# leavesnight/VIEO_SLAM

Measured on AMD Instinct MI355X. Metric: frontend+localBA frames/sec on EuRoC MH05 stereo-VIO; ATE vs ref, higher is better.
Workload: dtype u8 (extract/match) + f64 (pose optimisation)

## Files before the change

vieo_slam_amd/csrc/orb_extractor.hip:

```cpp
#include <algorithm>
#include <cmath>
#include <type_traits>
#include <vector>

#include "../../include/vieo_orb_pattern_31.h"
#include "common.h"
#include "sincosf_exact.h"
#include "wave_ops.h"

#define QT_DEVICE
#include "quadtree.inl"

#include "orb_internal.h"

namespace vieo {

#ifndef VIEO_RESIZE_ROWS
#define VIEO_RESIZE_ROWS 32
#endif
static const int kResizeRows = VIEO_RESIZE_ROWS;
#ifndef VIEO_QT_GROUPS
#define VIEO_QT_GROUPS {1, 64}
#endif

// ... 599 lines not shown
  int pitch;
  const uint8_t* src = plane_ptr(P, I, b, t.level, &pitch);
  const int ox = t.tx * kBlurTW, oy = t.ty * kBlurTH;
  const bool interior = ox >= 4 && ox + 68 <= D.w && oy >= 3 && oy + kBlurTH + 3 <= D.h &&
                        ((pitch & 3) == 0) && ((((uintptr_t)src) & 3) == 0);
  if (interior) {
    constexpr int NIT = (SH * (SP / 4) + 255) / 256;
    unsigned v[NIT];
#pragma unroll
    for (int k = 0; k < NIT; k++) {
      const int idx = tid + 256 * k, r = idx / (SP / 4), c4 = idx - r * (SP / 4);
      if (idx < SH * (SP / 4)) v[k] = *(const unsigned*)(src + (size_t)(oy + r - 3) * pitch + ox - 4 + 4 * c4);
    }
#pragma unroll
    for (int k = 0; k < NIT; k++)
      if (tid + 256 * k < SH * (SP / 4)) ((unsigned*)s_src)[tid + 256 * k] = v[k];
  } else {
    const bool aligned = ((pitch & 3) == 0) && ((((uintptr_t)src) & 3) == 0);
    constexpr int NIT = (SH * (SP / 4) + 255) / 256;
    unsigned v[NIT];
#pragma unroll
    for (int k = 0; k < NIT; k++) {
      const int idx = tid + 256 * k, r = idx / (SP / 4), c4 = idx - r * (SP / 4);
      v[k] = 0;
      if (idx < SH * (SP / 4)) {
        const int gy = reflect101(min(oy + r - 3, D.h + 2), D.h);
        const int gx0 = ox - 4 + 4 * c4;
        const uint8_t* row = src + (size_t)gy * pitch;
        if (aligned && gx0 >= 0 && gx0 + 4 <= D.w)
          v[k] = *(const unsigned*)(row + gx0);
        else {
#pragma unroll
          for (int j = 0; j < 4; j++) v[k] |= (unsigned)row[reflect101(min(gx0 + j, D.w + 2), D.w)] << (8 * j);
        }
      }
    }
#pragma unroll
    for (int k = 0; k < NIT; k++)
      if (tid + 256 * k < SH * (SP / 4)) ((unsigned*)s_src)[tid + 256 * k] = v[k];
  }
  __syncthreads();
  const unsigned K0123 = 18u | (34u << 8) | (48u << 16) | (56u << 24);
  const unsigned K456 = 48u | (34u << 8) | (18u << 16);
#ifndef VIEO_BLUR_AB
#define VIEO_BLUR_AB 0
#endif
  for (int idx = tid; idx < ((VIEO_BLUR_AB & 1) ? 0 : (SH / 2) * (kBlurTW / 4)); idx += 256) {
    const int pr = idx / (kBlurTW / 4), g = idx - pr * (kBlurTW / 4);
    unsigned h[2][4];
#pragma unroll
    for (int q = 0; q < 2; q++) {
      const unsigned* w = (const unsigned*)(s_src + (2 * pr + q) * SP) + g;
      const unsigned w0 = w[0], w1 = w[1], w2 = w[2];
      const unsigned a0 = __builtin_amdgcn_alignbyte(w1, w0, 1), b0 = __builtin_amdgcn_alignbyte(w2, w1, 1);
      const unsigned a1 = __builtin_amdgcn_alignbyte(w1, w0, 2), b1 = __builtin_amdgcn_alignbyte(w2, w1, 2);
      const unsigned a2 = __builtin_amdgcn_alignbyte(w1, w0, 3), b2 = __builtin_amdgcn_alignbyte(w2, w1, 3);
      h[q][0] = __builtin_amdgcn_udot4(b0, K456, __builtin_amdgcn_udot4(a0, K0123, 0u, false), false);
      h[q][1] = __builtin_amdgcn_udot4(b1, K456, __builtin_amdgcn_udot4(a1, K0123, 0u, false), false);
      h[q][2] = __builtin_amdgcn_udot4(b2, K456, __builtin_amdgcn_udot4(a2, K0123, 0u, false), false);
      h[q][3] = __builtin_amdgcn_udot4(w2, K456, __builtin_amdgcn_udot4(w1, K0123, 0u, false), false);
    }
    uint4 o;
    o.x = h[0][0] | (h[1][0] << 16), o.y = h[0][1] | (h[1][1] << 16);
    o.z = h[0][2] | (h[1][2] << 16), o.w = h[0][3] | (h[1][3] << 16);
    *(uint4*)(s_h + pr * kBlurTW + 4 * g) = o;
  }
  __syncthreads();
  typedef unsigned short us2 __attribute__((ext_vector_type(2)));
  uint8_t* dst = I.blur + (size_t)b * I.blur_img + D.boff;
  for (int idx = tid; idx < (kBlurTH / 2) * (kBlurTW / 4); idx += 256) {
    const int q = idx / (kBlurTW / 4), c4 = (idx - q * (kBlurTW / 4)) * 4;
    const int gy = oy + 2 * q, gx = ox + c4;
    if (gy >= D.h || gx >= D.w) continue;
#if VIEO_BLUR_AB & 1
    *(unsigned*)(dst + (size_t)gy * D.pitch + gx) = *(const unsigned*)(s_src + (2 * q + 3) * SP + c4 + 4);
    if (gy + 1 < D.h) *(unsigned*)(dst + (size_t)(gy + 1) * D.pitch + gx) = *(const unsigned*)(s_src + (2 * q + 4) * SP + c4 + 4);
    continue;
#endif
    const unsigned We[4] = {18u | (34u << 16), 48u | (56u << 16), 48u | (34u << 16), 18u};
    const unsigned Wo[4] = {18u << 16, 34u | (48u << 16), 56u | (48u << 16), 34u | (18u << 16)};
    unsigned e[4] = {1u << 15, 1u << 15, 1u << 15, 1u << 15}, o[4] = {1u << 15, 1u << 15, 1u << 15, 1u << 15};
#pragma unroll
    for (int k = 0; k < 4; k++) {
      const uint4 v = *(const uint4*)(s_h + (q + k) * kBlurTW + c4);
      const unsigned vv[4] = {v.x, v.y, v.z, v.w};
#pragma unroll
      for (int j = 0; j < 4; j++) {
        e[j] = __builtin_amdgcn_udot2(__builtin_bit_cast(us2, vv[j]), __builtin_bit_cast(us2, We[k]), e[j], false);
        o[j] = __builtin_amdgcn_udot2(__builtin_bit_cast(us2, vv[j]), __builtin_bit_cast(us2, Wo[k]), o[j], false);
      }
    }
    const unsigned oe = ((e[0] >> 16) & 0xFFu) | (((e[1] >> 16) & 0xFFu) << 8) | (((e[2] >> 16) & 0xFFu) << 16) |
                        (((e[3] >> 16) & 0xFFu) << 24);
    const unsigned oo = ((o[0] >> 16) & 0xFFu) | (((o[1] >> 16) & 0xFFu) << 8) | (((o[2] >> 16) & 0xFFu) << 16) |
                        (((o[3] >> 16) & 0xFFu) << 24);
    *(unsigned*)(dst + (size_t)gy * D.pitch + gx) = oe;
    if (gy + 1 < D.h) *(unsigned*)(dst + (size_t)(gy + 1) * D.pitch + gx) = oo;
  }
}

__device__ __forceinline__ int wave_sum(int v) { return wave_sum_i32(v); }

__device__ __forceinline__ float fast_atan2_deg(float y, float x) {
  const float p1 = 0.9997878412794807f * (float)(180 / 3.1415926535897932384626433832795);
  const float p3 = -0.3258083974640975f * (float)(180 / 3.1415926535897932384626433832795);
  const float p5 = 0.1555786518463281f * (float)(180 / 3.1415926535897932384626433832795);
  const float p7 = -0.04432655554792128f * (float)(180 / 3.1415926535897932384626433832795);
  const float eps = (float)2.2204460492503131e-16;
  const float ax = fabsf(x), ay = fabsf(y);
  float a, c, c2;
  if (ax >= ay) {
    c = ay / (ax + eps);
    c2 = c * c;
    a = (((p7 * c2 + p5) * c2 + p3) * c2 + p1) * c;
  } else {
    c = ax / (ay + eps);
    c2 = c * c;
    a = 90.f - (((p7 * c2 + p5) * c2 + p3) * c2 + p1) * c;
  }
  if (x < 0) a = 180.f - a;
  if (y < 0) a = 360.f - a;
  return a;
}

__global__ void __launch_bounds__(256)
k_desc_index(OrbParams P, const unsigned* __restrict__ sel, const int* __restrict__ sel_count,
             uint2* __restrict__ krec, int out_cap, int* __restrict__ counts) {
  const int b = blockIdx.y, g = blockIdx.x * 256 + threadIdx.x;
  int level = -1, idx = 0, total = 0;
  for (int l = 0; l < P.nlevels; l++) {
    const int n = max(sel_count[b * kMaxLevels + l], 0);
    if (level < 0 && g < total + n) {
      level = l;
      idx = g - total;
    }
    total += n;
  }
  if (g == 0) {
    counts[2 * b] = min(total, out_cap);
    counts[2 * b + 1] = 0;
  }
  if (g >= P.kp_cap) return;
  unsigned key = 0;
  if (level >= 0) key = sel[(size_t)b * P.sel_per_image + P.lv[level].sel_off + idx];
  krec[(size_t)b * P.kp_cap + g] = make_uint2(key, (unsigned)level);
}

#ifndef VIEO_DESC_KPW
#define VIEO_DESC_KPW 1
#endif
__global__ void __launch_bounds__(256)
k_describe(OrbParams P, ImgSet I, const uint2* __restrict__ krec, const int* __restrict__ pattern,
           vieo_keypoint* __restrict__ kp_out, uint8_t* __restrict__ desc_out, int out_cap,
           int groups_per_image, int n_images) {
  constexpr int KPW = VIEO_DESC_KPW;
  const int item = xcd_grouped(blockIdx.x, groups_per_image);
  const int b = item / groups_per_image;
  if (b >= n_images) return;
  const int lane = threadIdx.x & 63;
  const int wv = __builtin_amdgcn_readfirstlane((int)(threadIdx.x >> 6));
  const int g0 = ((item - b * groups_per_image) * (blockDim.x >> 6) + wv) * KPW;
  const int gmax = min(P.kp_cap, out_cap);
  if (g0 >= gmax) return;
  uint2 kr[KPW];
#pragma unroll
  for (int u = 0; u < KPW; u++) kr[u] = g0 + u < gmax ? krec[(size_t)b * P.kp_cap + g0 + u] : make_uint2(0, 0xFFFFFFFFu);
  constexpr int AP = 40, BR = 19, BP = 44;
  __shared__ __attribute__((aligned(16))) uint8_t s_patch[4][KPW][31 * AP + (2 * BR + 1) * BP];
  int pt4[4];
#pragma unroll
  for (int gq = 0; gq < 4; gq++) pt4[gq] = pattern[gq * 64 + lane];
  int cxs[KPW], cys[KPW], xas[KPW], xbs[KPW];
  unsigned va[KPW][8], vb[KPW][10];
  const int c = lane & 15, r0 = lane >> 4;
#pragma unroll
  for (int u = 0; u < KPW; u++) {
    const int level = (int)kr[u].y;
    if (level < 0) continue;
    const unsigned key = kr[u].x;
    const LevelDesc& D = P.lv[level];
    const int cx = QT_KEY_X(key) + (kEdge - 3), cy = QT_KEY_Y(key) + (kEdge - 3);
    int pitch;
    const uint8_t* img = plane_ptr(P, I, b, level, &pitch);
    const int xa = (cx - kHalfPatch) & ~3, xb = (cx - BR) & ~3;
    cxs[u] = cx, cys[u] = cy, xas[u] = xa, xbs[u] = xb;
    const uint8_t* bl0 = I.blur + (size_t)b * I.blur_img + D.boff;
    const int bp = D.pitch;
    const uint8_t* ga = img + (size_t)(cy - kHalfPatch + r0) * pitch + xa + 4 * c;
    const uint8_t* gb = bl0 + (size_t)(cy - BR + r0) * bp + xb + 4 * c;
#pragma unroll
    for (int k = 0; k < 8; k++)
      if (c < 9 && r0 + 4 * k < 31) va[u][k] = *(const unsigned*)(ga + (size_t)(4 * k) * pitch);
#pragma unroll
    for (int k = 0; k < 10; k++)
      if (c < 11 && r0 + 4 * k < 2 * BR + 1) vb[u][k] = *(const unsigned*)(gb + (size_t)(4 * k) * bp);
  }
#pragma unroll
  for (int u = 0; u < KPW; u++) {
    if ((int)kr[u].y < 0) continue;
    uint8_t* sa = s_patch[wv][u];
    uint8_t* sb = sa + 31 * AP;
#pragma unroll
    for (int k = 0; k < 8; k++)
      if (c < 9 && r0 + 4 * k < 31) *(unsigned*)(sa + (r0 + 4 * k) * AP + 4 * c) = va[u][k];
#pragma unroll
    for (int k = 0; k < 10; k++)
      if (c < 11 && r0 + 4 * k < 2 * BR + 1) *(unsigned*)(sb + (r0 + 4 * k) * BP + 4 * c) = vb[u][k];
  }
  __builtin_amdgcn_fence(__ATOMIC_ACQ_REL, "workgroup");
  __builtin_amdgcn_wave_barrier();
#pragma unroll
  for (int u = 0; u < KPW; u++) {
    const int level = (int)kr[u].y;
    if (level < 0) continue;
    const int g = g0 + u;
    const unsigned key = kr[u].x;
    const LevelDesc& D = P.lv[level];
    const int cx = cxs[u], cy = cys[u], xa = xas[u], xb = xbs[u];
    const uint8_t* sa = s_patch[wv][u];
    const uint8_t* sb = sa + 31 * AP;
    int m10 = 0, m01 = 0;
    if (lane < 62) {
      const int v = (lane >> 1) - kHalfPatch;
      const int d = P.umax[v < 0 ? -v : v];
      const uint8_t* row = sa + (v + kHalfPatch) * AP + (cx - xa);
      const int u0 = (lane & 1) ? 0 : -d, u1 = (lane & 1) ? d : -1;
      int sI = 0;
#pragma unroll
      for (int t = 0; t < 16; t++) {
        const int uu = u0 + t;
        if (uu <= u1) {
          const int val = row[uu];
          m10 += uu * val;
          sI += val;
        }
      }
      m01 = v * sI;
    }
    m10 = wave_sum(m10);
    m01 = wave_sum(m01);
    const float angle = fast_atan2_deg((float)m01, (float)m10);
    const float factorPI = (float)(3.1415926535897932384626433832795 / 180.f);
    float a, bsin;
    vieo_sincosf_exact(angle * factorPI, &bsin, &a);
    const uint8_t* bl = sb + BR * BP + (cx - xb);
    unsigned long long bits[4];
#pragma unroll
    for (int gq = 0; gq < 4; gq++) {
      const int pt = pt4[gq];
      const float x0 = (float)(signed char)(pt & 0xFF), y0 = (float)(signed char)((pt >> 8) & 0xFF);
      const float x1 = (float)(signed char)((pt >> 16) & 0xFF), y1 = (float)(signed char)((pt >> 24) & 0xFF);
      const int t0 = bl[__float2int_rn(x0 * bsin + y0 * a) * BP + __float2int_rn(x0 * a - y0 * bsin)];
      const int t1 = bl[__float2int_rn(x1 * bsin + y1 * a) * BP + __float2int_rn(x1 * a - y1 * bsin)];
      bits[gq] = __ballot(t0 < t1);
    }
    if (lane < 4) ((unsigned long long*)(desc_out + ((size_t)b * out_cap + g) * 32))[lane] = bits[lane];
    if (lane == 0) {
      vieo_keypoint k;
      const float fx = (float)cx, fy = (float)cy;
      k.x = level ? fx * D.scale : fx;
      k.y = level ? fy * D.scale : fy;
      k.size = (float)D.patch;
      k.angle = angle;
      k.response = (float)QT_KEY_R(key);
      k.octave = level;
      k.class_id = -1;
      kp_out[(size_t)b * out_cap + g] = k;
    }
  }
}

#ifndef VIEO_FUSED_AB
#define VIEO_FUSED_AB 0
#endif
constexpr int kFR = 18, kFRaw = kFR + 3;
constexpr int kFRawRows = 2 * kFRaw + 1, kFRawPitch = 48;
constexpr int kFHPairs = (kFRawRows + 1) / 2, kFHCols = 40;
constexpr int kFBlRows = 2 * kFR + 1, kFBlPitch = 40;
constexpr int kFWaveLds = kFRawRows * kFRawPitch + 16 + kFHPairs * kFHCols * 4;
static_assert(kFBlRows * kFBlPitch <= kFRawRows * kFRawPitch, "the blurred patch fits where the raw one was");

#ifndef VIEO_FUSED_KPW
#define VIEO_FUSED_KPW 4
#endif
static inline int fused_kpw(int n_images) { return n_images >= 32 ? VIEO_FUSED_KPW : 1; }
__global__ void __launch_bounds__(256)
k_describe_fused(OrbParams P, ImgSet I, const uint2* __restrict__ krec, const int* __restrict__ pattern,
                 vieo_keypoint* __restrict__ kp_out, uint8_t* __restrict__ desc_out, int out_cap,
                 int groups_per_image, int n_images, int KPW) {
  const int item = xcd_grouped(blockIdx.x, groups_per_image);
  const int b = item / groups_per_image;
  if (b >= n_images) return;
  const int lane = threadIdx.x & 63;
  const int wv = __builtin_amdgcn_readfirstlane((int)(threadIdx.x >> 6));
  const int g0 = ((item - b * groups_per_image) * (blockDim.x >> 6) + wv) * KPW;
  const int gmax = min(P.kp_cap, out_cap);
  if (g0 >= gmax) return;
  __shared__ __attribute__((aligned(16))) uint8_t s_all[4][kFWaveLds];
  int pt4[4];
#pragma unroll
  for (int gq = 0; gq < 4; gq++) pt4[gq] = pattern[gq * 64 + lane];
  uint8_t* s_raw = s_all[wv];
  unsigned* s_h = (unsigned*)(s_raw + kFRawRows * kFRawPitch + 16);
  constexpr int NLD = (kFRawRows + 3) / 4;
  unsigned v[NLD];
  bool interior = false;
  int sh = 0;
  const int c = lane & 15, r0 = lane >> 4;
  auto rec_of = [&](int u) { return (u < KPW && g0 + u < gmax) ? krec[(size_t)b * P.kp_cap + g0 + u] : make_uint2(0u, 0xFFFFFFFFu); };
  auto fetch = [&](const uint2 kr) {
    const int level = (int)kr.y;
    if (level < 0) return;
    const LevelDesc& D = P.lv[level];
    const int cx = QT_KEY_X(kr.x) + (kEdge - 3), cy = QT_KEY_Y(kr.x) + (kEdge - 3);
    int pitch;
    const uint8_t* img = plane_ptr(P, I, b, level, &pitch);
    const int x_lo = cx - kFRaw, y_lo = cy - kFRaw;
    const int xa = x_lo & ~3;
    sh = x_lo - xa;
    interior = x_lo >= 0 && y_lo >= 0 && cx + kFRaw < D.w && cy + kFRaw < D.h && xa + 52 <= pitch && ((pitch & 3) == 0) &&
               ((((uintptr_t)img) & 3) == 0);
    if (VIEO_FUSED_AB & 2) {
#pragma unroll
      for (int k = 0; k < NLD; k++) v[k] = kr.x + k;
      interior = false;
    } else if (interior) {
      const uint8_t* gp = img + (size_t)(y_lo + r0) * pitch + xa + 4 * c;
#pragma unroll
      for (int k = 0; k < NLD; k++) {
        v[k] = 0;
        if (c < 13 && r0 + 4 * k < kFRawRows) v[k] = *(const unsigned*)(gp + (size_t)(4 * k) * pitch);
      }
    } else {
#pragma unroll
      for (int k = 0; k < NLD; k++) {
        v[k] = 0;
        if (c < 12 && r0 + 4 * k < kFRawRows) {
          const uint8_t* row = img + (size_t)reflect101(min(max(y_lo + r0 + 4 * k, -(D.h - 1)), 2 * D.h - 2), D.h) * pitch;
#pragma unroll
          for (int jj = 0; jj < 4; jj++) {
            const int x = min(max(x_lo + 4 * c + jj, -(D.w - 1)), 2 * D.w - 2);
            v[k] |= (unsigned)row[reflect101(x, D.w)] << (8 * jj);
          }
        }
      }
    }
  };
  uint2 kr = rec_of(0);
  fetch(kr);
#pragma unroll 1
  for (int u = 0; u < KPW; u++) {
    const uint2 cur = kr;
    const int level = (int)cur.y;
    if (level < 0) break;
    const unsigned key = cur.x;
    const int g = g0 + u;
    const LevelDesc& D = P.lv[level];
    const int cx = QT_KEY_X(key) + (kEdge - 3), cy = QT_KEY_Y(key) + (kEdge - 3);
    if (interior) {
#pragma unroll
      for (int k = 0; k < NLD; k++) {
        const unsigned nxt = (unsigned)__builtin_amdgcn_update_dpp(0, (int)v[k], 0x101, 0xF, 0xF, false);
        v[k] = __builtin_amdgcn_alignbyte(nxt, v[k], sh);
      }
    }
#pragma unroll
    for (int k = 0; k < NLD; k++)
      if (c < 12 && r0 + 4 * k < kFRawRows) *(unsigned*)(s_raw + (r0 + 4 * k) * kFRawPitch + 4 * c) = v[k];
    __builtin_amdgcn_fence(__ATOMIC_ACQ_REL, "workgroup");
    __builtin_amdgcn_wave_barrier();
    kr = rec_of(u + 1);
    fetch(kr);
    {
      constexpr unsigned A0 = 18u | (34u << 8) | (48u << 16) | (56u << 24), A1 = 48u | (34u << 8) | (18u << 16);
      constexpr unsigned B0 = (18u << 8) | (34u << 16) | (48u << 24), B1 = 56u | (48u << 8) | (34u << 16) | (18u << 24);
      constexpr unsigned C0 = (18u << 16) | (34u << 24), C1 = 48u | (56u << 8) | (48u << 16) | (34u << 24), C2 = 18u;
      constexpr unsigned E0 = 18u << 24, E1 = 34u | (48u << 8) | (56u << 16) | (48u << 24), E2 = 34u | (18u << 8);
      for (int idx = lane; idx < ((VIEO_FUSED_AB & 1) ? 0 : kFHPairs * (kFHCols / 8)); idx += 64) {
        const int pr = idx / (kFHCols / 8), g8 = idx - pr * (kFHCols / 8);
        unsigned h[2][8];
#pragma unroll
        for (int q = 0; q < 2; q++) {
          const int r = min(2 * pr + q, kFRawRows - 1);
          const uint2* w = (const uint2*)(s_raw + r * kFRawPitch + 8 * g8);
          const uint2 lo = w[0], hi = w[1];
          const unsigned d0 = lo.x, d1 = lo.y, d2 = hi.x, d3 = hi.y;
#define DOT4(x, k, acc) __builtin_amdgcn_udot4(x, k, acc, false)
          h[q][0] = DOT4(d1, A1, DOT4(d0, A0, 0u));
          h[q][1] = DOT4(d1, B1, DOT4(d0, B0, 0u));
          h[q][2] = DOT4(d2, C2, DOT4(d1, C1, DOT4(d0, C0, 0u)));
          h[q][3] = DOT4(d2, E2, DOT4(d1, E1, DOT4(d0, E0, 0u)));
          h[q][4] = DOT4(d2, A1, DOT4(d1, A0, 0u));
          h[q][5] = DOT4(d2, B1, DOT4(d1, B0, 0u));
          h[q][6] = DOT4(d3, C2, DOT4(d2, C1, DOT4(d1, C0, 0u)));
          h[q][7] = DOT4(d3, E2, DOT4(d2, E1, DOT4(d1, E0, 0u)));
#undef DOT4
        }
        uint4 o0, o1;
        o0.x = h[0][0] | (h[1][0] << 16), o0.y = h[0][1] | (h[1][1] << 16);
        o0.z = h[0][2] | (h[1][2] << 16), o0.w = h[0][3] | (h[1][3] << 16);
        o1.x = h[0][4] | (h[1][4] << 16), o1.y = h[0][5] | (h[1][5] << 16);
        o1.z = h[0][6] | (h[1][6] << 16), o1.w = h[0][7] | (h[1][7] << 16);
        uint4* dst = (uint4*)(s_h + pr * kFHCols + 8 * g8);
        dst[0] = o0, dst[1] = o1;
      }
    }
    int m10 = 0, m01 = 0;
    if (lane < ((VIEO_FUSED_AB & 4) ? 1 : 62)) {
      const int vv = (lane >> 1) - kHalfPatch;
      const int d = P.umax[vv < 0 ? -vv : vv];
      const uint8_t* row = s_raw + (vv + kFRaw) * kFRawPitch + kFRaw;
      const int u0 = (lane & 1) ? 0 : -d, u1 = (lane & 1) ? d : -1;
      int sI = 0;
#pragma unroll
      for (int t = 0; t < 16; t++) {
        const int uu = u0 + t;
        if (uu <= u1) {
          const int val = row[uu];
          m10 += uu * val;
          sI += val;
        }
      }
      m01 = vv * sI;
    }
    m10 = wave_sum(m10);
    m01 = wave_sum(m01);
    const float angle = fast_atan2_deg((float)m01, (float)m10);
    __builtin_amdgcn_fence(__ATOMIC_ACQ_REL, "workgroup");
    __builtin_amdgcn_wave_barrier();
    typedef unsigned short us2 __attribute__((ext_vector_type(2)));
    uint8_t* s_bl = s_raw;
    for (int idx = lane; idx < ((VIEO_FUSED_AB & 1) ? 0 : ((kFBlRows + 1) / 2) * (kFBlPitch / 4)); idx += 64) {
      const int q = idx / (kFBlPitch / 4), c4 = (idx - q * (kFBlPitch / 4)) * 4;
      const unsigned We[4] = {18u | (34u << 16), 48u | (56u << 16), 48u | (34u << 16), 18u};
      const unsigned Wo[4] = {18u << 16, 34u | (48u << 16), 56u | (48u << 16), 34u | (18u << 16)};
      unsigned e[4] = {1u << 15, 1u << 15, 1u << 15, 1u << 15}, o[4] = {1u << 15, 1u << 15, 1u << 15, 1u << 15};
#pragma unroll
      for (int k = 0; k < 4; k++) {
        const uint4 hv = *(const uint4*)(s_h + (q + k) * kFHCols + c4);
        const unsigned vv[4] = {hv.x, hv.y, hv.z, hv.w};
#pragma unroll
        for (int jj = 0; jj < 4; jj++) {
          e[jj] = __builtin_amdgcn_udot2(__builtin_bit_cast(us2, vv[jj]), __builtin_bit_cast(us2, We[k]), e[jj], false);
          o[jj] = __builtin_amdgcn_udot2(__builtin_bit_cast(us2, vv[jj]), __builtin_bit_cast(us2, Wo[k]), o[jj], false);
        }
      }
      const unsigned oe = __builtin_amdgcn_perm(__builtin_amdgcn_perm(e[3], e[2], 0x0c0c0602u), __builtin_amdgcn_perm(e[1], e[0], 0x0c0c0602u), 0x05040100u);
      const unsigned oo = __builtin_amdgcn_perm(__builtin_amdgcn_perm(o[3], o[2], 0x0c0c0602u), __builtin_amdgcn_perm(o[1], o[0], 0x0c0c0602u), 0x05040100u);
      *(unsigned*)(s_bl + (2 * q) * kFBlPitch + c4) = oe;
      if (2 * q + 1 < kFBlRows) *(unsigned*)(s_bl + (2 * q + 1) * kFBlPitch + c4) = oo;
    }
    __builtin_amdgcn_fence(__ATOMIC_ACQ_REL, "workgroup");
    __builtin_amdgcn_wave_barrier();
    const float factorPI = (float)(3.1415926535897932384626433832795 / 180.f);
    float a, bsin;
    vieo_sincosf_exact(angle * factorPI, &bsin, &a);
    const uint8_t* bl = s_bl + kFR * kFBlPitch + kFR;
    unsigned long long bits[4];
#pragma unroll
    for (int gq = 0; gq < ((VIEO_FUSED_AB & 4) ? 1 : 4); gq++) {
      const int pt = pt4[gq];
      const float x0 = (float)(signed char)(pt & 0xFF), y0 = (float)(signed char)((pt >> 8) & 0xFF);
      const float x1 = (float)(signed char)((pt >> 16) & 0xFF), y1 = (float)(signed char)((pt >> 24) & 0xFF);
      const int t0 = bl[__float2int_rn(x0 * bsin + y0 * a) * kFBlPitch + __float2int_rn(x0 * a - y0 * bsin)];
      const int t1 = bl[__float2int_rn(x1 * bsin + y1 * a) * kFBlPitch + __float2int_rn(x1 * a - y1 * bsin)];
      bits[gq] = __ballot(t0 < t1);
    }
    if (lane < 4) ((unsigned long long*)(desc_out + ((size_t)b * out_cap + g) * 32))[lane] = bits[lane];
    if (lane == 0) {
      vieo_keypoint k;
      const float fx = (float)cx, fy = (float)cy;
      k.x = level ? fx * D.scale : fx;
      k.y = level ? fy * D.scale : fy;
      k.size = (float)D.patch;
      k.angle = angle;
      k.response = (float)QT_KEY_R(key);
      k.octave = level;
      k.class_id = -1;
      kp_out[(size_t)b * out_cap + g] = k;
    }
    __builtin_amdgcn_fence(__ATOMIC_ACQ_REL, "workgroup");
    __builtin_amdgcn_wave_barrier();
  }
}

__global__ void __launch_bounds__(256)
k_lapping(const vieo_keypoint* __restrict__ kin, const uint8_t* __restrict__ din, int in_cap,
          vieo_keypoint* __restrict__ kout, uint8_t* __restrict__ dout, int out_cap,
          const int* __restrict__ tmp_counts, int* __restrict__ counts, int lap0, int lap1) {
  __shared__ int s_part[256];
  __shared__ int s_total;
  const int b = blockIdx.x, tid = threadIdx.x;
  const int n = tmp_counts[2 * b];
  const int per = (n + 255) / 256;
  const int i0 = tid * per, i1 = min(n, i0 + per);
  int mono = 0;
  for (int i = i0; i < i1; i++) {
    const float x = kin[(size_t)b * in_cap + i].x;
    mono += !(x >= (float)lap0 && x <= (float)lap1);
  }
  s_part[tid] = mono;
  __syncthreads();
  if (tid == 0) {
    int acc = 0;
    for (int t = 0; t < 256; t++) {
      const int v = s_part[t];
      s_part[t] = acc;
      acc += v;
    }
    s_total = acc;
  }
  __syncthreads();
  int mi = s_part[tid];
  for (int i = i0; i < i1; i++) {
    const vieo_keypoint k = kin[(size_t)b * in_cap + i];
    const bool st = (k.x >= (float)lap0 && k.x <= (float)lap1);
    const int pos = st ? (n - 1 - (i - mi)) : mi;
    if (!st) mi++;
    if (pos < out_cap) {
      kout[(size_t)b * out_cap + pos] = k;
      const uint4* s = (const uint4*)(din + ((size_t)b * in_cap + i) * 32);
      uint4* d = (uint4*)(dout + ((size_t)b * out_cap + pos) * 32);
      d[0] = s[0];
      d[1] = s[1];
    }
  }
  if (tid == 0) {
    counts[2 * b] = min(n, out_cap);
    counts[2 * b + 1] = s_total;
  }
}

}

using namespace vieo;

namespace vieo {

static inline int cv_round_f(float v) { return (int)lrintf(v); }
static inline int cv_round_d(double v) { return (int)lrint(v); }
static inline int cv_floor_d(double v) {
  int i = (int)v;
  return i - (i > v);
}
static inline int cv_ceil_d(double v) {
  int i = (int)v;
  return i + (i < v);
}

static void resize_axis_table(int ssize, int dsize, bool horizontal, std::vector<short>& tab) {
  const double inv_scale = (double)dsize / ssize;
  const double sc = 1. / inv_scale;
  tab.resize((size_t)dsize * 4);
  for (int d = 0; d < dsize; d++) {
    float f = (float)((d + 0.5) * sc - 0.5);
    int s = cv_floor_d(f);
    f -= s;
    int s0, s1;
    if (horizontal) {
      if (s < 0) f = 0, s = 0;
      if (s >= ssize - 1) f = 0, s = ssize - 1;
      s0 = s;
      s1 = std::min(s + 1, ssize - 1);
    } else {
      s0 = std::min(std::max(s, 0), ssize - 1);
      s1 = std::min(std::max(s + 1, 0), ssize - 1);
    }
    short a0 = (short)cv_round_f((1.f - f) * 2048);
    short a1 = (short)cv_round_f(f * 2048);
    if (horizontal && s >= ssize - 1) a0 = 2048, a1 = 0;
    tab[d * 4 + 0] = (short)s0;
    tab[d * 4 + 1] = (short)s1;
    tab[d * 4 + 2] = a0;
    tab[d * 4 + 3] = a1;
  }
}

static int plan_geometry(vieo_orb* e, int w, int h, int B) {
  OrbParams& P = e->P;
  memset(&P, 0, sizeof(P));
  P.nlevels = e->nlevels;
  for (int i = 0; i <= kHalfPatch; i++) P.umax[i] = e->umax[i];
  e->cells.clear();
  e->tiles.clear();
  std::vector<short> xtab, ytab;
  int resize_rows = 1, resize_dw = 1;
  size_t pyr_off = 0, blur_off = 0;
  int max_cw = 0, max_ch = 0, key_off = 0, sel_off = 0, ncap_max = 0, max_ncell = 0;
  for (int l = 0; l < e->nlevels; l++) {
    LevelDesc& D = P.lv[l];
    const float s = e->inv_scale[l];
    D.w = cv_round_f((float)w * s);
    D.h = cv_round_f((float)h * s);
    if (D.w >= 4096 || D.h >= 4096) {
      set_error("image level %d (%dx%d) exceeds the 4095-pixel key packing", l, D.w, D.h);
      return VIEO_E_INVALID;
    }
    D.pitch = align_up(D.w, 16);
    if (l > 0) {
      D.off = (int)pyr_off;
      pyr_off += (size_t)D.pitch * D.h;
      pyr_off = align_up_sz(pyr_off, 256);
    }
    D.boff = (int)blur_off;
    blur_off += (size_t)D.pitch * D.h;
    blur_off = align_up_sz(blur_off, 256);
    D.nfeat = e->feats[l];
    D.scale = e->scale[l];
    D.patch = (int)(kPatchSize * e->scale[l]);
    const int minB = kEdge - 3;
    const int maxBX = D.w - kEdge + 3, maxBY = D.h - kEdge + 3;
    D.regW = maxBX - minB;
    D.regH = maxBY - minB;
    D.cell_begin = (int)e->cells.size();
    if (D.regW >= 35 && D.regH >= 35) {
      const float W = 35;
      const float width = (float)D.regW, height = (float)D.regH;
      const int nCols = (int)(width / W), nRows = (int)(height / W);
      const int wCell = (int)ceilf(width / nCols), hCell = (int)ceilf(height / nRows);
      for (int i = 0; i < nRows; i++) {
        const float iniY = minB + i * hCell;
        float maxY = iniY + hCell + 6;
        if (iniY >= maxBY - 3) continue;
        if (maxY > maxBY) maxY = maxBY;
        for (int j = 0; j < nCols; j++) {
          const float iniX = minB + j * wCell;
          float maxX = iniX + wCell + 6;
          if (iniX >= maxBX - 6) continue;
          if (maxX > maxBX) maxX = maxBX;
          CellDesc c;
          c.level = (short)l;
          c.x0 = (short)iniX, c.y0 = (short)iniY;
          c.cw = (short)((int)maxX - (int)iniX), c.ch = (short)((int)maxY - (int)iniY);
          c.offx = (short)(j * wCell), c.offy = (short)(i * hCell);
          c.pad = 0;
          e->cells.push_back(c);
          max_cw = std::max(max_cw, (int)c.cw);
          max_ch = std::max(max_ch, (int)c.ch);
        }
      }
      D.nIni = (int)roundf((float)D.regW / (float)D.regH);
      if (D.nIni < 1) {
        set_error("level %d region %dx%d too tall for DistributeOctTree (nIni=0)", l, D.regW, D.regH);
        return VIEO_E_INVALID;
      }
      D.hX = (float)D.regW / (float)D.nIni;
    } else {
      set_error("image too small: level %d is %dx%d", l, D.w, D.h);
      return VIEO_E_INVALID;
    }
    D.cell_end = (int)e->cells.size();
    max_ncell = std::max(max_ncell, D.cell_end - D.cell_begin);
    D.ncap = std::max(D.nfeat, 4 * D.nIni) + 8;
    ncap_max = std::max(ncap_max, D.ncap);
    D.sel_off = sel_off;
    sel_off += D.ncap;
    if (l > 0) {
      std::vector<short> t;
      D.xtab_off = (int)(xtab.size() / 4);
      resize_axis_table(P.lv[l - 1].w, D.w, true, t);
      xtab.insert(xtab.end(), t.begin(), t.end());
      D.ytab_off = (int)(ytab.size() / 4);
      resize_axis_table(P.lv[l - 1].h, D.h, false, t);
      ytab.insert(ytab.end(), t.begin(), t.end());
      const short* xt = xtab.data() + 4 * (size_t)D.xtab_off;
      const short* yt = ytab.data() + 4 * (size_t)D.ytab_off;
      for (int y0 = 0; y0 < D.h; y0 += kResizeRows)
        resize_rows = std::max(resize_rows, yt[4 * (std::min(y0 + kResizeRows, D.h) - 1) + 1] - yt[4 * y0] + 1);
      for (int x0 = 0; x0 < D.w; x0 += 256)
        resize_dw = std::max(resize_dw, ((xt[4 * (std::min(x0 + 256, D.w) - 1) + 1] + 4) >> 2) - (xt[4 * x0] >> 2));
    }
    D.tile_begin = (int)e->tiles.size();
    D.tiles_x = (D.w + kBlurTW - 1) / kBlurTW;
    for (int ty = 0; ty < (D.h + kBlurTH - 1) / kBlurTH; ty++)
      for (int tx = 0; tx < D.tiles_x; tx++) e->tiles.push_back({(short)l, (short)tx, (short)ty, 0});
    D.tile_end = (int)e->tiles.size();
  }
  P.ncells = (int)e->cells.size();
  if (max_cw - 6 > 64 || max_ch - 6 > 1023) {
    set_error("FAST cell wider than 64 pixels (image narrower than one 30-pixel cell?)");
    return VIEO_E_INVALID;
  }
  P.cell_cap = std::max(16, ((max_cw - 6 + 1) / 2) * ((max_ch - 6 + 1) / 2));
  for (int l = 0; l < e->nlevels; l++) {
    LevelDesc& D = P.lv[l];
    D.key_off = key_off;
    D.key_cap = (D.cell_end - D.cell_begin) * P.cell_cap;
    key_off += D.key_cap;
    if (D.key_cap >= (1 << 24)) {
      set_error("too many candidate keys per level");
      return VIEO_E_INVALID;
    }
  }
  P.keys_per_image = key_off;
  P.sel_per_image = sel_off;
  P.kp_cap = sel_off;
  e->ncap_max = ncap_max;
  e->scap_max = std::max(2 * ncap_max, max_ncell);
  e->pyr_img = align_up_sz(pyr_off, 256);
  e->blur_img = align_up_sz(blur_off, 256);
  e->resize_pitch = 4 * resize_dw + 4;
  e->resize_lds = resize_rows * e->resize_pitch;
  {
    bool ok = e->nlevels >= 3;
    int rows2 = 1, dw2 = 1;
    for (int l = 1; ok && l + 1 < e->nlevels; l += 2) {
      const LevelDesc &D1 = P.lv[l], &D2 = P.lv[l + 1];
      const short* xt1 = xtab.data() + 4 * (size_t)D1.xtab_off;
      const short* yt1 = ytab.data() + 4 * (size_t)D1.ytab_off;
      const short* xt2 = xtab.data() + 4 * (size_t)D2.xtab_off;
      const short* yt2 = ytab.data() + 4 * (size_t)D2.ytab_off;
      for (int ex0 = 0; ok && ex0 < D2.w; ex0 += kR2W) {
        const int ex1 = std::min(ex0 + kR2W, D2.w);
        const int rx0 = ex0 == 0 ? 0 : (xt2[4 * ex0] & ~3), rx1 = ex1 == D2.w ? D1.w : std::min(xt2[4 * (ex1 - 1) + 1] + 1, D1.w);
        const int ox1 = ex1 == D2.w ? D1.w : (xt2[4 * ex1] & ~3);
        const int ndw = ((xt1[4 * (rx1 - 1) + 1] + 4) >> 2) - ((xt1[4 * rx0] & ~3) >> 2);
        ok = rx1 - rx0 <= 256 && ox1 <= rx1 && ox1 > rx0 && ndw <= 128;
        dw2 = std::max(dw2, ndw);
      }
      for (int ey0 = 0; ok && ey0 < D2.h; ey0 += kR2H) {
        const int ey1 = std::min(ey0 + kR2H, D2.h);
        const int ry0 = ey0 == 0 ? 0 : yt2[4 * ey0], ry1 = ey1 == D2.h ? D1.h : std::min(yt2[4 * (ey1 - 1) + 1] + 1, D1.h);
        const int oy1 = ey1 == D2.h ? D1.h : yt2[4 * ey1];
        const int nrows = yt1[4 * (ry1 - 1) + 1] - yt1[4 * ry0] + 1;
        ok = ry1 - ry0 <= kR2Rows && oy1 <= ry1 && oy1 > ry0 && nrows <= 48;
        rows2 = std::max(rows2, nrows);
// ... 623 lines not shown
```

Baseline: 62120.

## Compute orientation moments with byte-perm masks and dot4, prefetch next keypoint record

Replaces the per-lane 16-iteration scalar loop for the intensity-centroid moments with precomputed byte-select masks, v_perm, udot4 and SAD instructions over five aligned LDS words. Keypoint records are now fetched two ahead and level descriptors are cached in registers, so the global pointer and stride computation no longer goes through plane_ptr. Address math is changed to a uniform base plus a per-lane 32-bit offset. This raises register pressure, and the mask construction depends on exact disc geometry (umax bounds, offsets 4/20), which could give wrong moments if misaligned.

```diff
diff --git a/vieo_slam_amd/csrc/orb_extractor.hip b/vieo_slam_amd/csrc/orb_extractor.hip
--- a/vieo_slam_amd/csrc/orb_extractor.hip
+++ b/vieo_slam_amd/csrc/orb_extractor.hip
@@ -925,60 +925,95 @@
   for (int gq = 0; gq < 4; gq++) pt4[gq] = pattern[gq * 64 + lane];
   uint8_t* s_raw = s_all[wv];
   unsigned* s_h = (unsigned*)(s_raw + kFRawRows * kFRawPitch + 16);
+  const int vv = min((lane >> 1) - kHalfPatch, kHalfPatch);
+  const bool odd = lane & 1;
+  unsigned dsel[4];
+  {
+    const int d = lane < ((VIEO_FUSED_AB & 4) ? 1 : 62) ? P.umax[vv < 0 ? -vv : vv] : -1;
+#pragma unroll
+    for (int k = 0; k < 4; k++) {
+      const int cnt = odd ? d + 1 - 4 * k : 16 - d - 4 * k;
+      const unsigned low = cnt >= 4 ? ~0u : cnt <= 0 ? 0u : (1u << (8 * cnt)) - 1u;
+      const unsigned keep = d < 0 ? 0u : odd ? low : ~low;
+      dsel[k] = (0x04030201u & keep) | (0x0c0c0c0cu & ~keep);
+    }
+  }
+  const uint8_t* disc_row = s_raw + (vv + kFRaw) * kFRawPitch + (odd ? 20 : 4);
   constexpr int NLD = (kFRawRows + 3) / 4;
   unsigned v[NLD];
   bool interior = false;
   int sh = 0;
   const int c = lane & 15, r0 = lane >> 4;
-  auto rec_of = [&](int u) { return (u < KPW && g0 + u < gmax) ? krec[(size_t)b * P.kp_cap + g0 + u] : make_uint2(0u, 0xFFFFFFFFu); };
-  auto fetch = [&](const uint2 kr) {
+  struct LvHead {
+    int w, h, pitch, off;
+    float scale;
+    int patch;
+  };
+  const uint2* krec_b = krec + (size_t)b * P.kp_cap + g0;
+  auto rec_of = [&](int u) {
+    uint2 r = krec_b[min(u, gmax - 1 - g0)];
+    if (!((u < KPW) & (g0 + u < gmax))) r.y = 0xFFFFFFFFu;
+    return r;
+  };
+  auto head_of = [&](const uint2 kr) {
+    const LevelDesc& D = P.lv[max((int)kr.y, 0)];
+    LvHead H;
+    H.w = D.w, H.h = D.h, H.pitch = D.pitch, H.off = D.off, H.scale = D.scale, H.patch = D.patch;
+    return H;
+  };
+  const uint8_t* img0_b = I.img0 + (size_t)b * I.img_pitch;
+  const uint8_t* pyr_b = I.pyr + (size_t)b * I.pyr_img;
+  auto fetch = [&](const uint2 kr, const LvHead& H) {
     const int level = (int)kr.y;
     if (level < 0) return;
-    const LevelDesc& D = P.lv[level];
     const int cx = QT_KEY_X(kr.x) + (kEdge - 3), cy = QT_KEY_Y(kr.x) + (kEdge - 3);
-    int pitch;
-    const uint8_t* img = plane_ptr(P, I, b, level, &pitch);
+    const int pitch = level ? H.pitch : I.stride0;
+    const uint8_t* img = level ? pyr_b + H.off : img0_b;
     const int x_lo = cx - kFRaw, y_lo = cy - kFRaw;
     const int xa = x_lo & ~3;
     sh = x_lo - xa;
-    interior = x_lo >= 0 && y_lo >= 0 && cx + kFRaw < D.w && cy + kFRaw < D.h && xa + 52 <= pitch && ((pitch & 3) == 0) &&
+    interior = (x_lo >= 0) & (y_lo >= 0) & (cx + kFRaw < H.w) & (cy + kFRaw < H.h) & (xa + 52 <= pitch) & ((pitch & 3) == 0) &
                ((((uintptr_t)img) & 3) == 0);
     if (VIEO_FUSED_AB & 2) {
 #pragma unroll
       for (int k = 0; k < NLD; k++) v[k] = kr.x + k;
       interior = false;
     } else if (interior) {
-      const uint8_t* gp = img + (size_t)(y_lo + r0) * pitch + xa + 4 * c;
+      const uint8_t* gp = img + (size_t)y_lo * pitch + xa;
+      const unsigned lane_off = (unsigned)(r0 * pitch + 4 * c);
 #pragma unroll
       for (int k = 0; k < NLD; k++) {
         v[k] = 0;
-        if (c < 13 && r0 + 4 * k < kFRawRows) v[k] = *(const unsigned*)(gp + (size_t)(4 * k) * pitch);
+        if (c < 13 && r0 + 4 * k < kFRawRows) v[k] = *(const unsigned*)(gp + (size_t)(4 * k) * pitch + lane_off);
       }
     } else {
 #pragma unroll
       for (int k = 0; k < NLD; k++) {
         v[k] = 0;
         if (c < 12 && r0 + 4 * k < kFRawRows) {
-          const uint8_t* row = img + (size_t)reflect101(min(max(y_lo + r0 + 4 * k, -(D.h - 1)), 2 * D.h - 2), D.h) * pitch;
+          const unsigned row = (unsigned)reflect101(min(max(y_lo + r0 + 4 * k, -(H.h - 1)), 2 * H.h - 2), H.h) * (unsigned)pitch;
 #pragma unroll
           for (int jj = 0; jj < 4; jj++) {
-            const int x = min(max(x_lo + 4 * c + jj, -(D.w - 1)), 2 * D.w - 2);
-            v[k] |= (unsigned)row[reflect101(x, D.w)] << (8 * jj);
+            const int x = min(max(x_lo + 4 * c + jj, -(H.w - 1)), 2 * H.w - 2);
+            v[k] |= (unsigned)img[row + (unsigned)reflect101(x, H.w)] << (8 * jj);
           }
         }
       }
     }
   };
-  uint2 kr = rec_of(0);
-  fetch(kr);
+  uint2 kr = rec_of(0), kr_next = rec_of(1);
+  LvHead H = head_of(kr);
+  fetch(kr, H);
 #pragma unroll 1
   for (int u = 0; u < KPW; u++) {
     const uint2 cur = kr;
     const int level = (int)cur.y;
     if (level < 0) break;
+    const LvHead D = H;
+    const uint2 kr_after = rec_of(u + 2);
+    H = head_of(kr_next);
     const unsigned key = cur.x;
     const int g = g0 + u;
-    const LevelDesc& D = P.lv[level];
     const int cx = QT_KEY_X(key) + (kEdge - 3), cy = QT_KEY_Y(key) + (kEdge - 3);
     if (interior) {
 #pragma unroll
@@ -992,8 +1027,8 @@
       if (c < 12 && r0 + 4 * k < kFRawRows) *(unsigned*)(s_raw + (r0 + 4 * k) * kFRawPitch + 4 * c) = v[k];
     __builtin_amdgcn_fence(__ATOMIC_ACQ_REL, "workgroup");
     __builtin_amdgcn_wave_barrier();
-    kr = rec_of(u + 1);
-    fetch(kr);
+    kr = kr_next, kr_next = kr_after;
+    fetch(kr, H);
     {
       constexpr unsigned A0 = 18u | (34u << 8) | (48u << 16) | (56u << 24), A1 = 48u | (34u << 8) | (18u << 16);
       constexpr unsigned B0 = (18u << 8) | (34u << 16) | (48u << 24), B1 = 56u | (48u << 8) | (34u << 16) | (18u << 24);
@@ -1028,23 +1063,18 @@
         dst[0] = o0, dst[1] = o1;
       }
     }
-    int m10 = 0, m01 = 0;
-    if (lane < ((VIEO_FUSED_AB & 4) ? 1 : 62)) {
-      const int vv = (lane >> 1) - kHalfPatch;
-      const int d = P.umax[vv < 0 ? -vv : vv];
-      const uint8_t* row = s_raw + (vv + kFRaw) * kFRawPitch + kFRaw;
-      const int u0 = (lane & 1) ? 0 : -d, u1 = (lane & 1) ? d : -1;
-      int sI = 0;
-#pragma unroll
-      for (int t = 0; t < 16; t++) {
-        const int uu = u0 + t;
-        if (uu <= u1) {
-          const int val = row[uu];
-          m10 += uu * val;
-          sI += val;
-        }
-      }
-      m01 = vv * sI;
+    int m10, m01;
+    {
+      const unsigned* rw = (const unsigned*)disc_row;
+      const unsigned w0 = rw[0], w1 = rw[1], w2 = rw[2], w3 = rw[3], w4 = rw[4];
+      const unsigned y0 = __builtin_amdgcn_perm(w1, w0, dsel[0]), y1 = __builtin_amdgcn_perm(w2, w1, dsel[1]);
+      const unsigned y2 = __builtin_amdgcn_perm(w3, w2, dsel[2]), y3 = __builtin_amdgcn_perm(w4, w3, dsel[3]);
+#define DOT4(x, k, acc) __builtin_amdgcn_udot4(x, k, acc, false)
+      const unsigned st = DOT4(y3, 0x0f0e0d0cu, DOT4(y2, 0x0b0a0908u, DOT4(y1, 0x07060504u, DOT4(y0, 0x03020100u, 0u))));
+      const unsigned sI = __builtin_amdgcn_sad_u8(y3, 0u, __builtin_amdgcn_sad_u8(y2, 0u, __builtin_amdgcn_sad_u8(y1, 0u, __builtin_amdgcn_sad_u8(y0, 0u, 0u))));
+#undef DOT4
+      m10 = odd ? (int)st : (int)st - 16 * (int)sI;
+      m01 = vv * (int)sI;
     }
     m10 = wave_sum(m10);
     m01 = wave_sum(m01);
```

New measurement: 62970, median of 6. 1.4% higher.
